# althonos/pyrodigal

Measured on AMD Instinct MI355X. Metric: Mbp/sec gene-called (meta mode), higher is better.
Workload: dtype f64; 1 GPU; 100000x20kbp_gc30-70_meta; contigs=100000, bases=2000000000, models=16, contigs_rank0=100000, sub_batch_contigs=6250, contexts_per_gpu=4, genes_all_ranks=2908995, steps_issued=a join of the contexts and a gather per step

## Files before the change

### pyrodigal_amd/csrc/finder.hip

```cpp
#include "pga_internal.h"
#include "pipeline.h"
#include "dpw_core.h"
#include "dev_common.h"

#include <math.h>
#include <stdio.h>
#include <stdlib.h>
#include <string.h>

#include <algorithm>
#include <atomic>
#include <chrono>
#include <condition_variable>
#include <functional>
#include <limits>
#include <map>
#include <memory>
#include <mutex>
#include <new>
#include <thread>
#include <type_traits>
#include <unordered_map>

namespace {
// ... 1511 lines not shown
                                  (int)batch->regions.size(), d_bits, d_mcounts, d_moff, d_miv, cap, st);
            HT(c, hipMemcpyAsync(h_moff_, d_moff, sizeof(int32_t) * (NC + 1), hipMemcpyDeviceToHost, st));
            h_moff = h_moff_; d_union_iv = d_miv;
            masks = MaskList{d_moff, d_miv};
        } else if (P.mask) {
            const int cap = (int)std::min<int64_t>(total / std::max(1, P.min_mask) + NC + 1, (int64_t)1 << 28);
            DEVBUF(d_runs, MaskRun, "d_mask_runs", cap + 1);
            DEVBUF(d_nruns, int32_t, "d_mask_count", 4);
            DEVBUF(d_moff, int32_t, "d_mask_off", NC + 2);
            DEVBUF(d_miv, int2, "d_mask_iv", cap + 1);
            pga_launch_find_masks(d_dig, d_ct, NC, batch->d_tiles, batch->n_tiles, P.min_mask, d_runs, d_nruns, cap, st);
            int32_t nruns = 0;
            HT(c, hipMemcpyAsync(&nruns, d_nruns, 4, hipMemcpyDeviceToHost, st));
            HT(c, hipStreamSynchronize(st));
            nruns = std::min(nruns, cap);
            std::vector<MaskRun> runs((size_t)nruns);
            if (nruns > 0) HT(c, hipMemcpy(runs.data(), d_runs, sizeof(MaskRun) * nruns, hipMemcpyDeviceToHost));
            std::sort(runs.begin(), runs.end(), [](const MaskRun& a, const MaskRun& b) { return a.contig != b.contig ? a.contig < b.contig : a.begin < b.begin; });
            std::vector<int32_t> moff(NC + 1, 0);
            std::vector<int2> miv((size_t)nruns + 1);
            for (int k = 0; k < nruns; k++) { moff[runs[k].contig + 1]++; miv[k] = make_int2(runs[k].begin, runs[k].end); }
            for (int i = 0; i < NC; i++) moff[i + 1] += moff[i];
            R->mask_off = moff;
            R->masks.resize(2 * (size_t)nruns);
            for (int k = 0; k < nruns; k++) { R->masks[2 * k] = runs[k].begin; R->masks[2 * k + 1] = runs[k].end; }
            HT(c, hipMemcpy(d_moff, moff.data(), sizeof(int32_t) * (NC + 1), hipMemcpyHostToDevice));
            if (nruns > 0) HT(c, hipMemcpy(d_miv, miv.data(), sizeof(int2) * nruns, hipMemcpyHostToDevice));
            masks = MaskList{d_moff, d_miv};
        }
        if (stage == PGA_STAGE_SEQUENCE) {
            HT(c, hipMemcpyAsync(h_cnt, d_cnt, sizeof(int32_t) * 2 * (size_t)NC, hipMemcpyDeviceToHost, st));
            HT(c, hipGetLastError());
            HT(c, hipStreamSynchronize(st));
            for (int i = 0; i < NC; i++) {
                R->contigs[i].gc = ct[i].len > 0 ? (double)h_cnt[i] / (double)ct[i].len : 0.0;
                R->contigs[i].n_unknown = h_cnt[NC + i];
            }
            if (h_moff) { const int rc = fetch_mask_union(c, R, h_moff, d_union_iv, NC); if (rc) return rc; }
            return publish(R, guard.r, P, out);
        }
        if (meta_run && NM > 0 && use_sets) {
            DEVBUF(d_set_of, int32_t, "d_set_of", 3 * (size_t)NC + 1);
            HT(c, hipMemcpyAsync(d_set_of, set_of.data(), sizeof(int32_t) * (size_t)NC, hipMemcpyHostToDevice, st));
            pga_launch_group_enable_sets(d_ct, NC, d_cnt, d_set_of, d_set_of + NC, f->d_model_gc, f->d_model_grp, NM, NG, d_enabled, st);
        } else if (meta_run && NM > 0) {
            pga_launch_group_enable(d_ct, NC, d_cnt, f->d_model_gc, f->d_model_grp, NM, NG, d_enabled, st);
        }
        if (multi) {
            for (int g = 0; g < NG; g++) for (int i = 0; i < NC; i++) h_enabled[(size_t)g * NC + i] = cgrp[i] == g;
            HT(c, hipMemcpyAsync(d_enabled, h_enabled, (size_t)NG * NC, hipMemcpyHostToDevice, st));
        }
        if (getenv("PGA_STAGE_FULL")) f->stage_full = true;
        bool stage_full = f->stage_full;
        c->extract_passes = 0;
        for (;;) {
            const bool half = !stage_full;
            const int shift = half ? std::max(1, std::min(8, getenv("PGA_STAGE_SHIFT") ? atoi(getenv("PGA_STAGE_SHIFT")) : 1)) : 0;
            const int64_t st_slots = half ? (total >> shift) + (int64_t)PGA_STAGE_SLACK * batch->n_tiles + 8 : 2 * total + 2;
            for (int g = 0; g < NG; g++) {
                char nm[32];
                GBUF(st_ndx, int32_t, st_slots) GBUF(st_sv, int32_t, st_slots) GBUF(st_info, uint8_t, st_slots)
                ga[g].st_half = shift; ga[g].st_overflow = d_st_overflow;
            }
            if (c->extract_passes > 0) HT(c, hipMemsetAsync(d_st_overflow, 0, sizeof(int32_t), st));
            for (int g = 0; g < NG; g++) {
                const int tt = meta_run ? f->group_tt[g] : multi ? gtt[g] : (stage == PGA_STAGE_EXTRACT ? tt_override : c->models[0].trans_table);
                pga_launch_extract(d_dig, total, d_ct, NC, tt, P, ga[g], batch->d_tiles, batch->n_tiles, batch->d_tile0, d_tile_first, d_tile_last,
                                   d_tile_count + (size_t)g * (batch->n_tiles + 1), d_tile_off + (size_t)g * (batch->n_tiles + 1), d_cbase + (size_t)g * (NC + 1),
                                   d_tile_scount + (size_t)g * (batch->n_tiles + 1), d_tile_soff + (size_t)g * (batch->n_tiles + 1), d_sbase + (size_t)g * (NC + 1),
                                   masks, st, ((meta_run && NM > 0) || multi) ? d_enabled + (size_t)g * NC : nullptr);
            }
            HT(c, hipMemcpyAsync(h_xa, d_xa, sizeof(int32_t) * xa_words, hipMemcpyDeviceToHost, st));
            HT(c, hipGetLastError());
            HT(c, hipStreamSynchronize(st));
            c->extract_passes++;
            if (!half || h_st_overflow[0] == 0) break;
            stage_full = true;
            if (!getenv("PGA_STAGE_SHIFT")) f->stage_full = true;
        }
        if (h_moff) { const int rc = fetch_mask_union(c, R, h_moff, d_union_iv, NC); if (rc) return rc; }

        tm.mark("extract+sync");
        int64_t group_nodes[4] = {0, 0, 0, 0};
        for (int g = 0; g < NG; g++) {
            char nm[32];
            group_nodes[g] = h_cbase[(size_t)g * (NC + 1) + NC];
            const int64_t n = group_nodes[g] + 1;
            GBUF(ndx, int32_t, n) GBUF(stop_val, int32_t, n) GBUF(type, uint8_t, n) GBUF(strand, int8_t, n) GBUF(edge0, uint8_t, n) GBUF(gc_cont, float, n) GBUF(contig_of, int32_t, n)
            GBUF(stop_list, int32_t, (int64_t)h_sbase[(size_t)g * (NC + 1) + NC] + 1)
            GBUF(start_list, int32_t, group_nodes[g] - (int64_t)h_sbase[(size_t)g * (NC + 1) + NC] + 1)
            GBUF(ovl_topo, uint32_t, (int64_t)h_sbase[(size_t)g * (NC + 1) + NC] + 1)
            GBUF(srank, int32_t, n + 4)
        }
        for (int g = 0; g < NG; g++) {
            pga_launch_place(d_ct, batch->d_tiles, batch->n_tiles, d_tile_off + (size_t)g * (batch->n_tiles + 1),
                             d_tile_soff + (size_t)g * (batch->n_tiles + 1), ga[g], st);
            pga_launch_orf_gc(d_ct, NC, d_dig, d_p16, ga[g], (int)group_nodes[g], d_cbase + (size_t)g * (NC + 1), st);
        }
        std::vector<std::vector<ChainDesc>> gch(NG);
        std::vector<double> mgc((size_t)NM); std::vector<int> mtt((size_t)NM);
        for (int m = 0; m < NM; m++) { mgc[m] = c->models[m].gc; mtt[m] = c->models[m].trans_table; }
        for (int g = 0; g < NG; g++) gch[g].reserve(meta_run ? (size_t)NC * 6 : (size_t)NC);
        std::vector<double> set_gc;
        if (use_sets) {
            std::vector<int64_t> sum((size_t)2 * NS, 0);
            for (int i = 0; i < NC; i++) { sum[2 * (size_t)set_of[i]] += h_cnt[i]; sum[2 * (size_t)set_of[i] + 1] += ct[i].len; }
            set_gc.resize((size_t)NS);
            for (int s = 0; s < NS; s++) set_gc[(size_t)s] = sum[2 * (size_t)s + 1] > 0 ? (double)sum[2 * (size_t)s] / (double)sum[2 * (size_t)s + 1] : 0.0;
        }
        for (int i = 0; i < NC; i++) {
            const int L = ct[i].len;
            double gc = L > 0 ? (double)h_cnt[i] / (double)L : 0.0;
            R->contigs[i].gc = gc;
            R->contigs[i].n_unknown = h_cnt[NC + i];
            if (!meta_run) {
                const int m = per_contig ? model_of_contig[i] : 0, g = multi ? cgrp[i] : 0;
                const int32_t* cb = h_cbase + (size_t)g * (NC + 1);
                ChainDesc ch{0, cb[i], cb[i + 1] - cb[i], m, i, 1};
                ch.group = g;
                gch[g].push_back(ch);
                continue;
            }
            if (use_sets) gc = set_gc[(size_t)set_of[i]];
            const double low = fmin(0.65, 0.88495 * gc - 0.0102337), high = fmax(0.35, 0.86596 * gc + 0.1131991);
            int tt_prev = -1;
            for (int m = 0; m < NM; m++) {
                if (mgc[m] < low || mgc[m] > high) continue;
                const int g = f->model_group[m];
                if (!h_enabled[(size_t)g * NC + i]) { c->err = "pga_find_genes: host and device disagree on a GC window"; return PGA_EDEVICE; }
                const int32_t* cb = h_cbase + (size_t)g * (NC + 1);
                ChainDesc ch{0, cb[i], cb[i + 1] - cb[i], m, i, mtt[m] != tt_prev ? 1 : 0};
// ... 1058 lines not shown
```

### pyrodigal_amd/csrc/pipeline.h

```cpp
#pragma once
#include "pga_internal.h"

struct ContigDesc {
    int64_t base;
    int32_t len;
    int32_t _pad;
};

#define PGA_STAGE_SLACK 8
struct TileDesc {
    int32_t contig;
    int32_t start;
};

struct GroupArrays {
    uint8_t* df;
    int32_t* c16; const int32_t* tile0 = nullptr;
    int32_t* st_ndx; int32_t* st_sv;
    uint8_t* st_info;
    int32_t st_half = 0; int32_t* st_overflow = nullptr;
    int32_t* stop_list;
    int32_t* start_list = nullptr;
    uint32_t* ovl_topo;
    int32_t* srank = nullptr;
    int32_t* ndx; int32_t* stop_val; uint8_t* type; int8_t* strand; uint8_t* edge0; float* gc_cont;
    int32_t* contig_of = nullptr;
};

struct ChainArrays {
    double* cscore; double* sscore; double* rscore; double* uscore; double* tscore; double* mot_score;
    double* cscore_raw;
    int32_t* star_ptr;
    int32_t* mot_ndx;
    uint8_t* rbs;
    uint8_t* edge;
    uint8_t* mot_len; uint8_t* mot_spacer; uint8_t* mot_spacendx;
    double* cs_sink = nullptr;
};

struct ModelScoreConst {
    double lfac_min, lfac_max;
    double lfac_tab[1001];
};

struct MaskList {
    const int32_t* off;
    const int2* iv;
};
struct MaskRun { int32_t contig, begin, end, _pad; };

struct ScoreParams {
    int32_t closed, is_meta, max_overlap, n_models;
    double* cs_out;
    uint8_t* conv_flag;
    unsigned long long* prof = nullptr;
    int32_t models_per_pass = 512;
    int32_t lean_stops = 0;
};

void pga_launch_digitize(const char* d_seq, uint8_t* d_dig, int64_t total, const ContigDesc* d_ct, int n_contigs,
                         int32_t* d_gc, int32_t* d_unk, hipStream_t st);
int64_t pga_gc_blocks(int64_t total);
void pga_launch_gc_prefix(const uint8_t* d_dig, int64_t total, int32_t* d_block_sum, int32_t* d_block_off, int32_t* d_p16, hipStream_t st);
void pga_launch_extract(const uint8_t* d_dig, int64_t total, const ContigDesc* d_ct, int n_contigs, int tt,
                        const pga_params& p, const GroupArrays& ga, const TileDesc* d_tiles, int n_tiles, const int32_t* d_tile0,
                        int32_t* d_tile_first, int32_t* d_tile_last, int32_t* d_tile_count, int32_t* d_tile_off, int32_t* d_cbase,
                        int32_t* d_tile_scount, int32_t* d_tile_soff, int32_t* d_sbase ,
                        MaskList masks, hipStream_t st,
                        const uint8_t* d_enabled = nullptr );
void pga_launch_place(const ContigDesc* d_ct, const TileDesc* d_tiles, int n_tiles, const int32_t* d_tile_off, const int32_t* d_tile_soff,
                      const GroupArrays& ga, hipStream_t st);
struct StopLaunch {
    const int32_t* sbase = nullptr;
    int64_t soff_begin = 0, n_pairs = 0;
    int32_t n_stops = 0;
    const int32_t* topo_q2 = nullptr; void* ext = nullptr;
    bool fill_star_ptr = true;
    bool starts_only = false; int32_t n_starts = 0;
    const int32_t* blk_chain = nullptr;
    void* mm_rec = nullptr;
    void* mm_chain = nullptr;
    void* mm_tile = nullptr;
    void* mm_scratch = nullptr;
    int32_t mm_tiles = 0;
};
int pga_mm_tile_items();
int32_t pga_mm_tiles(const ChainDesc* h_chains, int n_chains, const int32_t* h_cbase, const int32_t* h_sbase, int n_models, std::vector<int64_t>& scratch);
size_t pga_mm_scratch_bytes(int n_models, int n_chains);
constexpr size_t PGA_SS_REC_BYTES = 32, PGA_SS_MMCHAIN_BYTES = 32, PGA_SS_MMTILE_BYTES = 16;
void pga_launch_group_enable(const ContigDesc* d_ct, int n_contigs, const int32_t* d_gc_count, const double* d_model_gc,
                             const int32_t* d_model_group, int n_models, int n_groups, uint8_t* d_enabled, hipStream_t st);
void pga_launch_group_enable_sets(const ContigDesc* d_ct, int n_contigs, const int32_t* d_gc_count, const int32_t* d_set_of, int32_t* d_pool,
                                  const double* d_model_gc, const int32_t* d_model_group, int n_models, int n_groups, uint8_t* d_enabled,
                                  hipStream_t st);
void pga_launch_find_masks(const uint8_t* d_dig, const ContigDesc* d_ct, int n_contigs, const TileDesc* d_tiles, int n_tiles, int min_mask,
                           MaskRun* d_runs, int32_t* d_count, int cap, hipStream_t st);
int64_t pga_mask_words(int64_t total);
int64_t pga_mask_waves(int64_t total);
void pga_launch_mask_union(const uint8_t* d_dig, const char* d_seq, int64_t total, const ContigDesc* d_ct, int n_contigs, const TileDesc* d_tiles,
                           int n_tiles, int unknown_runs, int lower_case_runs, int min_mask, const MaskRun* d_regions, int n_regions,
                           uint32_t* d_bits, int32_t* d_counts, int32_t* d_moff, int2* d_miv, int cap, hipStream_t st);
int pga_extract_tile_size();
void pga_launch_orf_gc(const ContigDesc* d_ct, int n_contigs, const uint8_t* d_dig, const int32_t* d_p16, const GroupArrays& ga,
                       int n_nodes_total, const int32_t* d_node_contig_base, hipStream_t st);
void pga_launch_score(const ChainDesc* d_chains, int n_chains, int64_t node_begin, int64_t total, const uint8_t* d_dig,
                      const ContigDesc* d_ct, const GroupArrays& ga, const pga_training* d_models,
                      const ModelScoreConst* d_msc, const ModelConst* d_mc, const ChainArrays& ca, ScoreParams sp,
                      const ChainDesc* d_all_chains , const int2* d_contig_chains ,
                      const int32_t* d_node_contig_base, int n_contigs, int group_nodes, const unsigned* d_sd_lut, hipStream_t st,
                      int reuse_raw_cscore = 0 ,
                      const double* d_gil = nullptr , int il_stride = 0,
                      const int32_t* d_rank = nullptr ,
                      const void* d_cs_tasks = nullptr, int n_cs_tasks = 0, const void* d_cs_entries = nullptr ,
                      const StopLaunch* stops = nullptr);
bool pga_cs_tasks(const int2* h_cc, int n_contigs, const ChainDesc* h_chains, const int32_t* h_cbase, const int32_t* model_rank, int task_nodes,
                  std::vector<int32_t>& tasks, std::vector<int32_t>& entries);
void pga_launch_sd_lut(unsigned* d_lut, hipStream_t st);
```

### pyrodigal_amd/csrc/pipeline.hip

```cpp

#include "pga_internal.h"
#include "pipeline.h"
#include <atomic>
#include "dev_common.h"
#include "dpw_core.h"

namespace {

enum { NA = 0, NG = 1, NC = 2, NT = 3, NN = 6 };

__device__ __forceinline__ int find_contig(const ContigDesc* __restrict__ ct, int n, int64_t g) {
    int lo = 0, hi = n - 1;
    while (lo < hi) { int mid = (lo + hi + 1) >> 1; if (ct[mid].base <= g) lo = mid; else hi = mid - 1; }
    return lo;
}

__device__ __forceinline__ int block_contig(const ContigDesc* __restrict__ ct, int n, int64_t block_first, int64_t g, int* s_slot) {
    int c = block_search_le([&](const int k) { return ct[k].base; }, n, block_first, s_slot);
    while (c + 1 < n && ct[c + 1].base <= g) c++;
    return c;
}
__device__ __forceinline__ int block_chain(const ChainDesc* __restrict__ ch, int n, int64_t block_first, int64_t g, int* s_slot) {
    int c = block_search_le([&](const int k) { return ch[k].off; }, n, block_first, s_slot);
    while (c + 1 < n && ch[c + 1].off <= g) c++;
// ... 108 lines not shown
            int a = in ? gc : 0, u = in ? unk : 0;
#pragma unroll
            for (int m = 32; m >= 1; m >>= 1) { a += __shfl_xor(a, m, 64); u += __shfl_xor(u, m, 64); }
            if (acc_c != c0) {
                if ((threadIdx.x & 63) == 0 && acc_c >= 0) { if (acc_gc) atomicAdd(&gc_count[acc_c], acc_gc); if (acc_unk) atomicAdd(&unk_count[acc_c], acc_unk); }
                acc_c = c0; acc_gc = 0; acc_unk = 0;
            }
            acc_gc += a; acc_unk += u;
        } else if (in && one_contig) {
            if (gc) atomicAdd(&gc_count[c], gc);
            if (unk) atomicAdd(&unk_count[c], unk);
        }
    }
    __shared__ int s_c[4], s_g[4], s_u[4];
    const int wv = threadIdx.x >> 6;
    if ((threadIdx.x & 63) == 0) { s_c[wv] = acc_c; s_g[wv] = acc_gc; s_u[wv] = acc_unk; }
    __syncthreads();
    if (threadIdx.x == 0) {
#pragma unroll
        for (int w = 0; w < 4; w++) {
            if (s_c[w] < 0) continue;
            int g = s_g[w], u = s_u[w];
#pragma unroll
            for (int v = w + 1; v < 4; v++) if (s_c[v] == s_c[w]) { g += s_g[v]; u += s_u[v]; s_c[v] = -1; }
            if (g) atomicAdd(&gc_count[s_c[w]], g);
            if (u) atomicAdd(&unk_count[s_c[w]], u);
        }
    }
}

constexpr int EX_TILE = 3072;
constexpr int EX_PER_THREAD = 12;
constexpr int EX_NONE_HI = 0x7fffffff;

__device__ __forceinline__ unsigned pack4(const unsigned w, const bool comp) {
    unsigned c = w & 0x03030303u;
    if (comp) { const unsigned nm = (w >> 2) & 0x01010101u; c = (c ^ 0x03030303u) ^ (nm | (nm << 1)); }
    return (c | (c >> 6) | (c >> 12) | (c >> 18)) & 0xffu;
}
__device__ __forceinline__ unsigned long long pack16(const uint4 v, const bool comp) {
    return (unsigned long long)(pack4(v.x, comp) | (pack4(v.y, comp) << 8) | (pack4(v.z, comp) << 16) | (pack4(v.w, comp) << 24));
}
__device__ __forceinline__ unsigned long long pairrev64(unsigned long long x) {
    x = __brevll(x);
    return ((x & 0x5555555555555555ull) << 1) | ((x >> 1) & 0x5555555555555555ull);
}

struct TileGeom {
    int L, a, len;
    __device__ __forceinline__ int lo(const int strand) const { return strand == 1 ? a : L - a - len; }
};
__device__ __forceinline__ TileGeom tile_geom(const TileDesc td, const int L) { return TileGeom{L, td.start, min(EX_TILE, L - td.start)}; }

struct ExShared {
    int lsc[3][256];
    int scm[256];
    int32_t sv[2][EX_PER_THREAD][256];
    int wmin[3][4], wmax[3][4], wlsc[3][4];
    int carry_ns[3], carry_ps[3];
    int wsum[4];
};

struct ExParams { int tt, closed, min_gene, min_edge_gene; unsigned long long stop_codons, start_codons; };

__device__ __forceinline__ unsigned pairrev32(unsigned x) {
    x = __brev(x);
    return ((x & 0x55555555u) << 1) | ((x >> 1) & 0x55555555u);
}
__device__ __forceinline__ unsigned unknown4(const unsigned w) {
    const unsigned n = (w >> 2) & 0x01010101u;
    return (n | (n >> 7) | (n >> 14) | (n >> 21)) & 0xfu;
}

template <int STRAND>
__device__ __forceinline__ void strand_codon_masks(const TileGeom G, const uint8_t* __restrict__ d, const int64_t base, const int64_t total, const int i0,
                                                   const unsigned long long stop_codons, const unsigned long long start_codons,
                                                   unsigned& inm, unsigned& cw, unsigned& stm, unsigned& scm) {
    constexpr bool FWD = STRAND == 1;
    const int L = G.L, lo = G.lo(STRAND), end = lo + G.len;
    const int qa = max(0, lo - i0), qb = min(EX_PER_THREAD - 1, min(end - 1, L - 3) - i0);
    inm = qb >= qa ? ((2u << qb) - 1u) & ~((1u << qa) - 1u) : 0u;
    cw = 0; unsigned unk = 0xffffu;
    if (inm) {
        const int64_t ga0 = FWD ? base + i0 : base + (L - 1 - i0 - 15);
        if (ga0 >= 0 && ga0 <= total) {
            uint4 v; __builtin_memcpy(&v, (FWD ? d + i0 : d + (L - 1 - i0 - 15)), 16);
            const unsigned q0 = (unsigned)pack16(v, !FWD);
            const unsigned n0 = unknown4(v.x) | (unknown4(v.y) << 4) | (unknown4(v.z) << 8) | (unknown4(v.w) << 12);
            cw = FWD ? q0 : pairrev32(q0);
            unk = FWD ? n0 : (__brev(n0) >> 16);
        } else {
            unk = 0;
            for (int q = 0; q < 16; q++) {
                const int i = i0 + q;
                const int b = (i >= 0 && i < L) ? sbase(d, L, i, STRAND) : NN;
                if (b > 3) unk |= 1u << q; else cw |= (unsigned)b << (2 * q);
            }
        }
        if (i0 < 0) unk |= (1u << min(16, -i0)) - 1u;
        if (i0 + 16 > L) unk |= ~((1u << max(0, L - i0)) - 1u) & 0xffffu;
    }
    stm = 0; scm = 0;
#pragma unroll
    for (int q = 0; q < EX_PER_THREAD; q++) {
        const unsigned idx = (cw >> (2 * q)) & 63u;
        stm |= ((unsigned)(stop_codons >> idx) & 1u) << q;
        scm |= ((unsigned)(start_codons >> idx) & 1u) << q;
    }
    const unsigned okm = inm & ~(unk | (unk >> 1) | (unk >> 2));
    stm &= okm; scm &= okm;
}

template <int STRAND>
__device__ __forceinline__ void extract_strand(ExShared& S, const TileGeom G, const uint8_t* __restrict__ d, const int64_t base, const int64_t total,
                                               const int tile, const TileDesc* __restrict__ tiles, const int n_tiles,
                                               const int32_t* __restrict__ tile_first, const int32_t* __restrict__ tile_last, const ExParams P,
                                               const int n_masks, const int2* __restrict__ mv, unsigned& nodes, unsigned long long& infos) {
    constexpr bool FWD = STRAND == 1;
    const int t = threadIdx.x, lane = t & 63, w = t >> 6, L = G.L, s = FWD ? 0 : 1;
    const int lo = G.lo(STRAND), end = lo + G.len;
    const int top = FWD ? G.a : L - 1 - G.a - (EX_PER_THREAD - 1);
    const int i0 = FWD ? top + t * EX_PER_THREAD : top - t * EX_PER_THREAD;
    const int f0 = ((top % 3) + 3) % 3;
    nodes = 0; infos = 0;
    if (t < 6) {
        const int f = t % 3;
        const int64_t so = (int64_t)s * n_tiles;
        const int contig = tiles[tile].contig;
        const int up = FWD ? 1 : -1;
        if (t < 3) {
            int v = EX_NONE_HI;
            for (int k = tile + up; k >= 0 && k < n_tiles && tiles[k].contig == contig; k += up) {
                v = tile_first[(so + k) * 3 + f];
                if (v != EX_NONE_HI) break;
            }
            S.carry_ns[f] = v;
        } else {
            int v = -1;
            for (int k = tile - up; k >= 0 && k < n_tiles && tiles[k].contig == contig; k -= up) {
                v = tile_last[(so + k) * 3 + f];
                if (v != -1) break;
            }
            S.carry_ps[f] = v;
        }
    }
    unsigned inm, cw, stm, scm;
    strand_codon_masks<STRAND>(G, d, base, total, i0, P.stop_codons, P.start_codons, inm, cw, stm, scm);
    int mn[3], mx[3], ls[3];
#pragma unroll
    for (int r = 0; r < 3; r++) {
        const unsigned fr = 0x249u << r;
        const unsigned a = stm & fr, b = scm & fr;
        mn[r] = a ? i0 + __builtin_ctz(a) : EX_NONE_HI;
        mx[r] = a ? i0 + 31 - __builtin_clz(a) : -1;
        ls[r] = b ? i0 + 31 - __builtin_clz(b) : -1;
    }
    const unsigned long long lanes_up = FWD ? (~1ull << lane) : ((1ull << lane) - 1ull);
    const unsigned long long lanes_dn = FWD ? ((1ull << lane) - 1ull) : (~1ull << lane);
    int xa[3], xb[3], xe[3];
#pragma unroll
    for (int r = 0; r < 3; r++) {
        const unsigned long long hs = __ballot(mx[r] >= 0), hc = __ballot(ls[r] >= 0);
        const unsigned long long mu = hs & lanes_up, md = hs & lanes_dn, mc = hc & lanes_dn;
        const int su = mu ? (FWD ? __builtin_ctzll(mu) : 63 - __builtin_clzll(mu)) : lane;
        const int sd = md ? (FWD ? 63 - __builtin_clzll(md) : __builtin_ctzll(md)) : lane;
        const int sc = mc ? (FWD ? 63 - __builtin_clzll(mc) : __builtin_ctzll(mc)) : lane;
        const int va = __shfl(mn[r], su, 64), vb = __shfl(mx[r], sd, 64), ve = __shfl(ls[r], sc, 64);
        xa[r] = mu ? va : EX_NONE_HI;
        xb[r] = md ? vb : -1;
        xe[r] = ls[r] >= 0 ? ls[r] : (mc ? ve : -1);
        const int l_first = hs ? (FWD ? __builtin_ctzll(hs) : 63 - __builtin_clzll(hs)) : 0;
        const int l_last = hs ? (FWD ? 63 - __builtin_clzll(hs) : __builtin_ctzll(hs)) : 0;
        const int l_lastc = hc ? (FWD ? 63 - __builtin_clzll(hc) : __builtin_ctzll(hc)) : 0;
        const int w_mn = __shfl(mn[r], l_first, 64), w_mx = __shfl(mx[r], l_last, 64), w_ls = __shfl(ls[r], l_lastc, 64);
        if (lane == 0) { S.wmin[r][w] = hs ? w_mn : EX_NONE_HI; S.wmax[r][w] = hs ? w_mx : -1; S.wlsc[r][w] = hc ? w_ls : -1; }
    }
    S.scm[t] = (int)scm;
    __syncthreads();
    int nxt[3], prv[3];
#pragma unroll
    for (int r = 0; r < 3; r++) {
        int a = xa[r], b = xb[r], e = xe[r];
#pragma unroll
        for (int k = 0; k < 4; k++) {
            const bool up_side = FWD ? k > w : k < w, dn_side = FWD ? k < w : k > w;
            if (up_side) a = min(a, S.wmin[r][k]);
            if (dn_side) { b = max(b, S.wmax[r][k]); e = max(e, S.wlsc[r][k]); }
        }
        const int f = (f0 + r) % 3;
        nxt[r] = a == EX_NONE_HI ? S.carry_ns[f] : a;
        prv[r] = b == -1 ? S.carry_ps[f] : b;
        S.lsc[r][t] = e;
    }
    __syncthreads();
    auto mask_bound = [&](const int last) -> int {
        if (n_masks <= 0) return INT_MIN;
        if (FWD) {
            int a = 0, b = n_masks;
            while (a < b) { const int m = (a + b) >> 1; if (mv[m].x <= last) a = m + 1; else b = m; }
            if (a > 0) { const int2 m = mv[a - 1]; if (m.x < last) return m.y; }
        } else {
            const int x = L - last - 1;
            int a = 0, b = n_masks;
            while (a < b) { const int m = (a + b) >> 1; if (mv[m].y < x) a = m + 1; else b = m; }
            if (a < n_masks) { const int2 m = mv[a]; if (x < m.y) return L - 1 - m.x; }
        }
        return INT_MIN;
    };
    auto last_start_codon = [&](const int r, const int f, const int x, const int lower) -> int {
        int y;
        if (x >= lo) {
            const int tx = FWD ? (x - top) / EX_PER_THREAD : (top + EX_PER_THREAD - 1 - x) / EX_PER_THREAD;
            const int i0x = FWD ? top + tx * EX_PER_THREAD : top - tx * EX_PER_THREAD;
            const unsigned m = (unsigned)S.scm[tx] & ((2u << (x - i0x)) - 1u) & (0x249u << r);
            if (m) return i0x + 31 - __builtin_clz(m);
            const int nb = FWD ? tx - 1 : tx + 1;
            const int v = (nb >= 0 && nb < 256) ? S.lsc[r][nb] : -1;
            if (v >= 0) return v;
            y = lo - 1 - ((lo - 1 - f) % 3 + 3) % 3;
        } else y = x - ((x - f) % 3 + 3) % 3;
        for (int i = y; i >= lower && i >= 0; i -= 3)
            if (codon_is_start(sbase(d, L, i, STRAND), sbase(d, L, i + 1, STRAND), sbase(d, L, i + 2, STRAND), P.tt)) return i;
        return -1;
    };
    auto orf_has_start = [&](const int r, const int f, const int last, const int left, const bool real) -> bool {
        const int mb = mask_bound(last);
        const int lower = max(left + 1, mb);
        const int mind = real ? P.min_gene : P.min_edge_gene;
        const int x = min(last + 3 - mind, last - 3);
        if (x >= lower && last_start_codon(r, f, x, lower) >= lower) return true;
        return !P.closed && left < 0 && f < last && last - f > P.min_edge_gene && f >= mb;
    };
    auto put = [&](const int q, const int info, const int sv) {
        const int k = FWD ? q : EX_PER_THREAD - 1 - q;
        nodes |= 1u << k;
        infos |= (unsigned long long)info << (4 * k);
        S.sv[s][k][t] = sv;
    };
    unsigned cand = stm | scm;
    if (!P.closed) {
        if (i0 <= 2 && i0 + EX_PER_THREAD > 0) cand |= (i0 >= 0 ? 7u >> i0 : 7u << -i0) & inm;
#pragma unroll
        for (int r = 0; r < 3; r++) {
            const int f = (f0 + r) % 3;
            const int q = (L - 3 - ((L - 3 - f) % 3)) - i0;
            if (q >= 0 && q < EX_PER_THREAD) cand |= (1u << q) & inm;
        }
    }
    auto candidate = [&](const int q, const bool is_stop) {
        const int i = i0 + q;
        const int r = q % 3, f = (f0 + r) % 3;
        const unsigned fr = 0x249u << r;
        const unsigned above = stm & fr & ~((2u << q) - 1u);
        const unsigned below = stm & fr & ((1u << q) - 1u);
        const int left = below ? i0 + 31 - __builtin_clz(below) : (r == 0 ? prv[0] : (r == 1 ? prv[1] : prv[2]));
        const int sv_stop = FWD ? (left >= 0 ? left : f - 6) : (left >= 0 ? L - 1 - left : L - f + 5);
        if (is_stop) {
            if (orf_has_start(r, f, i, left, true)) put(q, PGA_T_STOP, sv_stop);
            return;
        }
        int last = above ? i0 + __builtin_ctz(above) : (r == 0 ? nxt[0] : (r == 1 ? nxt[1] : nxt[2]));
        const bool real = last != EX_NONE_HI;
        if (!real) {
            if (P.closed) return;
            last = L - 3 - ((L - 3 - f) % 3);
            if (last < i) return;
            if (last == i) {
                if (orf_has_start(r, f, i, left, false)) put(q, PGA_T_STOP | (1 << 2), sv_stop);
                return;
            }
        }
        if (n_masks > 0 && i < mask_bound(last)) return;
        const int mind = real ? P.min_gene : P.min_edge_gene;
        int type = -1, edge = 0;
        const int c0 = (int)((cw >> (2 * q)) & 3u);
        if (last - i + 3 >= mind && ((scm >> q) & 1u)) type = c0 == NA ? 0 : (c0 == NT ? 2 : 1);
        else if (i <= 2 && !P.closed && last - i > P.min_edge_gene) { type = 0; edge = 1; }
        if (type < 0) return;
        put(q, type | (edge << 2), FWD ? last : L - 1 - last);
    };
    unsigned stops = stm;
    while (stops) { const int q = __builtin_ctz(stops); stops &= stops - 1u; candidate(q, true); }
    cand &= ~stm;
    while (cand) { const int q = __builtin_ctz(cand); cand &= cand - 1u; candidate(q, false); }
}

__global__ void __launch_bounds__(64)
k_tile_stops(const uint8_t* __restrict__ dig, int64_t total, const ContigDesc* __restrict__ ct, const TileDesc* __restrict__ tiles, int n_tiles,
             unsigned long long stop_codons, int32_t* __restrict__ tile_first, int32_t* __restrict__ tile_last, const uint8_t* __restrict__ enabled) {
    const TileDesc td = tiles[blockIdx.x];
    if (enabled != nullptr && !enabled[td.contig]) return;
    const ContigDesc cd = ct[td.contig];
    const TileGeom G = tile_geom(td, cd.len);
    const int lane = threadIdx.x & 63, hl = lane & 31;
    const bool first = lane < 32;
    const uint8_t* __restrict__ d = dig + cd.base;
    constexpr int CHUNK = 32 * EX_PER_THREAD;
#pragma unroll
    for (int s = 0; s < 2; s++) {
        const int lo = G.lo(s == 0 ? 1 : -1), end = lo + G.len;
        int res[3];
        res[0] = res[1] = res[2] = first ? EX_NONE_HI : -1;
        unsigned found = 0;
        int fbase = 0;
        for (int c = 0; c * CHUNK < G.len && found != 63u; c++) {
            const int i0 = first ? lo + c * CHUNK + hl * EX_PER_THREAD : end - c * CHUNK - (hl + 1) * EX_PER_THREAD;
            fbase = ((i0 % 3) + 3) % 3;
            unsigned inm, cw, stm, scm;
            if (s == 0) strand_codon_masks<1>(G, d, cd.base, total, i0, stop_codons, 0ull, inm, cw, stm, scm);
            else strand_codon_masks<-1>(G, d, cd.base, total, i0, stop_codons, 0ull, inm, cw, stm, scm);
#pragma unroll
            for (int r = 0; r < 3; r++) {
                const unsigned m = stm & (0x249u << r);
                const unsigned long long hs = __ballot(m != 0u);
                const unsigned h_first = (unsigned)hs, h_last = (unsigned)(hs >> 32);
                const int v = m ? (first ? i0 + __builtin_ctz(m) : i0 + 31 - __builtin_clz(m)) : 0;
                const int src = first ? (h_first ? __builtin_ctz(h_first) : 0) : (h_last ? 32 + __builtin_ctz(h_last) : 32);
                const int wv = __shfl(v, src, 64);
                const bool mine_has = first ? h_first != 0u : h_last != 0u;
                const unsigned bit = first ? (1u << r) : (8u << r);
                if (mine_has && !(found & bit)) res[r] = wv;
                found |= (h_first ? (1u << r) : 0u) | (h_last ? (8u << r) : 0u);
            }
        }
        if (hl < 3) {
            const int f = (fbase + hl) % 3;
            const int64_t o = ((int64_t)s * n_tiles + blockIdx.x) * 3 + f;
            const int v = hl == 0 ? res[0] : (hl == 1 ? res[1] : res[2]);
            if (first) tile_first[o] = v; else tile_last[o] = v;
        }
    }
}

__global__ void __launch_bounds__(256)
k_extract_tile(const uint8_t* __restrict__ dig, int64_t total, const ContigDesc* __restrict__ ct, const TileDesc* __restrict__ tiles, int n_tiles,
               const int32_t* __restrict__ tile_first, const int32_t* __restrict__ tile_last, ExParams P, GroupArrays ga, MaskList masks,
               const uint8_t* __restrict__ enabled, int32_t* __restrict__ tile_count, int32_t* __restrict__ tile_scount) {
    __shared__ ExShared S;
    __shared__ int s_stops;
    const int tile = blockIdx.x, t = threadIdx.x;
    const TileDesc td = tiles[tile];
    if (enabled != nullptr && !enabled[td.contig]) { if (t == 0) { tile_count[tile] = 0; tile_scount[tile] = 0; } return; }
    if (t == 0) s_stops = 0;
    const ContigDesc cd = ct[td.contig];
    const TileGeom G = tile_geom(td, cd.len);
    const uint8_t* __restrict__ d = dig + cd.base;
    const int n_masks = masks.off ? masks.off[td.contig + 1] - masks.off[td.contig] : 0;
    const int2* __restrict__ mv = masks.off ? masks.iv + masks.off[td.contig] : nullptr;
    unsigned nf, nr; unsigned long long inf_f, inf_r;
    extract_strand<1>(S, G, d, cd.base, total, tile, tiles, n_tiles, tile_first, tile_last, P, n_masks, mv, nf, inf_f);
    __syncthreads();
    extract_strand<-1>(S, G, d, cd.base, total, tile, tiles, n_tiles, tile_first, tile_last, P, n_masks, mv, nr, inf_r);
    const int r0 = t * EX_PER_THREAD;
    const int cnt = __popc(nf) + __popc(nr);
    int inc = cnt;
    const int lane = t & 63, w = t >> 6;
#pragma unroll
    for (int off = 1; off < 64; off <<= 1) { const int v = __shfl_up(inc, off, 64); if (lane >= off) inc += v; }
    if (lane == 63) S.wsum[w] = inc;
    __syncthreads();
    int nbase = inc - cnt;
    for (int k = 0; k < w; k++) nbase += S.wsum[k];
    if (t == 255) tile_count[tile] = nbase + cnt;
    const int64_t g0 = cd.base + G.a;
    if (r0 < G.len) {
        const int nk = min(EX_PER_THREAD, G.len - r0);
        auto spread4 = [](const unsigned x) { return ((x & 15u) * 0x00204081u) & 0x01010101u; };
        if (nk == EX_PER_THREAD) {
            unsigned w[3];
            __builtin_memcpy(w, dig + g0 + r0, 12);
#pragma unroll
            for (int q = 0; q < 3; q++) w[q] = (w[q] & 0x07070707u) | (spread4(nf >> (4 * q)) << 4) | (spread4(nr >> (4 * q)) << 5);
            __builtin_memcpy(ga.df + g0 + r0, w, 12);
        } else {
            for (int k = 0; k < nk; k++) ga.df[g0 + r0 + k] = (uint8_t)((dig[g0 + r0 + k] & 7u) | (((nf >> k) & 1u) << 4) | (((nr >> k) & 1u) << 5));
        }
    }
    const int64_t stage0 = ga.st_half ? (g0 >> ga.st_half) + (int64_t)PGA_STAGE_SLACK * tile : 2 * g0;
    const int room = ga.st_half ? (G.len >> ga.st_half) + PGA_STAGE_SLACK : 2 * G.len;
    if (t == 255 && nbase + cnt > room) atomicOr(ga.st_overflow, 1);
    int64_t slot = stage0 + nbase;
    const int64_t slot_end = stage0 + room;
    unsigned both = nf | nr;
    int n_stop = 0;
    while (both) {
        const int k = __builtin_ctz(both);
        both &= both - 1u;
        if ((nf >> k) & 1u) {
            const int info = (int)((inf_f >> (4 * k)) & 7);
            if (slot < slot_end) { ga.st_ndx[slot] = G.a + r0 + k; ga.st_sv[slot] = S.sv[0][k][t]; ga.st_info[slot] = (uint8_t)info; }
            slot++; n_stop += (info & 3) == PGA_T_STOP;
        }
        if ((nr >> k) & 1u) {
            const int info = (int)((inf_r >> (4 * k)) & 7);
            if (slot < slot_end) { ga.st_ndx[slot] = G.a + r0 + k; ga.st_sv[slot] = S.sv[1][k][t]; ga.st_info[slot] = (uint8_t)(info | 8); }
            slot++; n_stop += (info & 3) == PGA_T_STOP;
        }
    }
#pragma unroll
    for (int m = 32; m >= 1; m >>= 1) n_stop += __shfl_xor(n_stop, m, 64);
    if (lane == 0 && n_stop) atomicAdd(&s_stops, n_stop);
    __syncthreads();
    if (t == 0) tile_scount[tile] = s_stops;
}

constexpr int SCAN_E = 4;
__device__ __forceinline__ int scan_pad(const int i) { return i + (i >> 5); }
__global__ void __launch_bounds__(1024)
k_scan_counts(const int32_t* __restrict__ cnt, int n, int32_t* __restrict__ off, const int32_t* __restrict__ cnt2, int32_t* __restrict__ off2) {
    __shared__ int s_a[SCAN_E * 1024 + SCAN_E * 32], s_b[SCAN_E * 1024 + SCAN_E * 32];
    __shared__ int s_w[16], s_w2[16];
    __shared__ int s_carry, s_carry2;
    const int t = threadIdx.x, lane = t & 63, w = t >> 6;
    const bool two = cnt2 != nullptr;
    if (t == 0) { s_carry = 0; s_carry2 = 0; }
    __syncthreads();
    for (int base = 0; base < n; base += SCAN_E * 1024) {
        int c[SCAN_E], c2[SCAN_E];
#pragma unroll
        for (int k = 0; k < SCAN_E; k++) {
            const int g = base + k * 1024 + t;
            c[k] = g < n ? cnt[g] : 0;
            c2[k] = two && g < n ? cnt2[g] : 0;
        }
#pragma unroll
        for (int k = 0; k < SCAN_E; k++) { s_a[scan_pad(k * 1024 + t)] = c[k]; s_b[scan_pad(k * 1024 + t)] = c2[k]; }
        __syncthreads();
        int v[SCAN_E], v2[SCAN_E], sum = 0, sum2 = 0;
#pragma unroll
        for (int k = 0; k < SCAN_E; k++) { v[k] = s_a[scan_pad(t * SCAN_E + k)]; v2[k] = s_b[scan_pad(t * SCAN_E + k)]; sum += v[k]; sum2 += v2[k]; }
        int inc = sum, inc2 = sum2;
#pragma unroll
        for (int o = 1; o < 64; o <<= 1) {
            const int x = __shfl_up(inc, o, 64), x2 = __shfl_up(inc2, o, 64);
            if (lane >= o) { inc += x; inc2 += x2; }
        }
        if (lane == 63) { s_w[w] = inc; s_w2[w] = inc2; }
        __syncthreads();
        int run = s_carry + inc - sum, run2 = s_carry2 + inc2 - sum2;
        for (int k = 0; k < w; k++) { run += s_w[k]; run2 += s_w2[k]; }
#pragma unroll
        for (int k = 0; k < SCAN_E; k++) {
            s_a[scan_pad(t * SCAN_E + k)] = run; s_b[scan_pad(t * SCAN_E + k)] = run2;
            run += v[k]; run2 += v2[k];
        }
        __syncthreads();
#pragma unroll
        for (int k = 0; k < SCAN_E; k++) {
// ... 2133 lines not shown
#pragma unroll
    for (int o = 1; o < 64; o <<= 1) {
        const int x = __shfl_up(is, o, 64), y = __shfl_up(ie, o, 64);
        if (lane >= o) { is += x; ie += y; }
    }
    if (!(S | E)) return;
    int ks = off_s[w >> 6] + is - ns, ke = off_e[w >> 6] + ie - ne;
    while (S) {
        const int64_t g = w * 32 + __builtin_ctz(S);
        S &= S - 1u;
        if (ks < cap) iv[ks].x = (int)(g - ct[find_contig(ct, n_contigs, g)].base);
        ks++;
    }
    while (E) {
        const int64_t g = w * 32 + __builtin_ctz(E);
        E &= E - 1u;
        if (ke < cap) iv[ke].y = (int)(g + 1 - ct[find_contig(ct, n_contigs, g)].base);
        ke++;
    }
}

int64_t pga_mask_words(int64_t total) { return (total + 32) / 32; }
int64_t pga_mask_waves(int64_t total) { return (pga_mask_words(total) + 63) / 64; }

void pga_launch_mask_union(const uint8_t* d_dig, const char* d_seq, int64_t total, const ContigDesc* d_ct, int n_contigs, const TileDesc* d_tiles,
                           int n_tiles, int unknown_runs, int lower_case_runs, int min_mask, const MaskRun* d_regions, int n_regions,
                           uint32_t* d_bits, int32_t* d_counts, int32_t* d_moff, int2* d_miv, int cap, hipStream_t st) {
    const int64_t nw = pga_mask_words(total), nwv = pga_mask_waves(total);
    uint32_t* const d_cbits = d_bits + nw;
    int32_t* const cnt_s = d_counts; int32_t* const cnt_e = cnt_s + (nwv + 1); int32_t* const off_s = cnt_e + (nwv + 1); int32_t* const off_e = off_s + (nwv + 1);
    (void)hipMemsetAsync(d_bits, 0, sizeof(uint32_t) * 2 * (size_t)nw, st);
    const dim3 run_grid(n_tiles + (n_contigs + 255) / 256);
    if (unknown_runs) hipLaunchKernelGGL(k_mask_paint_runs<RunOfUnknown>, run_grid, dim3(256), 0, st, d_dig, d_ct, d_tiles, n_tiles, n_contigs, min_mask, d_bits);
    if (lower_case_runs) hipLaunchKernelGGL(k_mask_paint_runs<RunOfLowerCase>, run_grid, dim3(256), 0, st, (const uint8_t*)d_seq, d_ct, d_tiles, n_tiles, n_contigs, min_mask, d_bits);
    hipLaunchKernelGGL(k_mask_paint_regions, dim3((n_regions + 3) / 4 + (n_contigs + 255) / 256), dim3(256), 0, st, d_regions, n_regions, d_ct, n_contigs, d_bits, d_cbits);
    const int word_blocks = (int)((nw + 255) / 256);
    hipLaunchKernelGGL(k_mask_count, dim3(word_blocks), dim3(256), 0, st, (const uint32_t*)d_bits, (const uint32_t*)d_cbits, nw, cnt_s, cnt_e);
    hipLaunchKernelGGL(k_scan_counts, dim3(1), dim3(1024), 0, st, (const int32_t*)cnt_s, (int)nwv, off_s, (const int32_t*)cnt_e, off_e);
    hipLaunchKernelGGL(k_mask_place, dim3(word_blocks + (n_contigs + 1 + 255) / 256), dim3(256), 0, st, (const uint32_t*)d_bits, (const uint32_t*)d_cbits, nw, word_blocks,
                       (const int32_t*)off_s, (const int32_t*)off_e, d_ct, n_contigs, d_moff, d_miv, cap);
}

void pga_launch_gc_prefix(const uint8_t* d_dig, int64_t total, int32_t* d_block_sum, int32_t* d_block_off, int32_t* d_p16, hipStream_t st) {
    if (total <= 0) return;
    const int nb = (int)pga_gc_blocks(total);
    hipLaunchKernelGGL(k_gcp_blocks, dim3(nb), dim3(256), 0, st, d_dig, total, d_block_sum);
    hipLaunchKernelGGL(k_scan_counts, dim3(1), dim3(1024), 0, st, d_block_sum, nb, d_block_off, (const int32_t*)nullptr, (int32_t*)nullptr);
    hipLaunchKernelGGL(k_gcp_final, dim3(nb), dim3(256), 0, st, d_dig, total, d_block_off, d_p16);
}

void pga_launch_extract(const uint8_t* d_dig, int64_t total, const ContigDesc* d_ct, int n_contigs, int tt,
                        const pga_params& p, const GroupArrays& ga, const TileDesc* d_tiles, int n_tiles, const int32_t* d_tile0,
                        int32_t* d_tile_first, int32_t* d_tile_last, int32_t* d_tile_count, int32_t* d_tile_off, int32_t* d_cbase,
                        int32_t* d_tile_scount, int32_t* d_tile_soff, int32_t* d_sbase, MaskList masks, hipStream_t st, const uint8_t* d_enabled) {
    if (n_tiles > 0) {
        ExParams P{tt, p.closed, p.min_gene, p.min_edge_gene, 0ull, 0ull};
        for (int idx = 0; idx < 64; idx++) {
            const int b0 = idx & 3, b1 = (idx >> 2) & 3, b2 = (idx >> 4) & 3;
            if (codon_is_stop(b0, b1, b2, tt)) P.stop_codons |= 1ull << idx;
            if (codon_is_start(b0, b1, b2, tt)) P.start_codons |= 1ull << idx;
        }
        hipLaunchKernelGGL(k_tile_stops, dim3(n_tiles), dim3(64), 0, st, d_dig, total, d_ct, d_tiles, n_tiles, P.stop_codons, d_tile_first, d_tile_last, d_enabled);
        hipLaunchKernelGGL(k_extract_tile, dim3(n_tiles), dim3(256), 0, st, d_dig, total, d_ct, d_tiles, n_tiles, d_tile_first, d_tile_last, P, ga, masks,
                           d_enabled, d_tile_count, d_tile_scount);
    }
    hipLaunchKernelGGL(k_scan_counts, dim3(1), dim3(1024), 0, st, d_tile_count, n_tiles, d_tile_off, (const int32_t*)d_tile_scount, d_tile_soff);
    hipLaunchKernelGGL(k_contig_node_base, dim3((n_contigs + 1 + 255) / 256), dim3(256), 0, st, d_tile0, n_contigs, d_tile_off, d_cbase);
    hipLaunchKernelGGL(k_contig_node_base, dim3((n_contigs + 1 + 255) / 256), dim3(256), 0, st, d_tile0, n_contigs, d_tile_soff, d_sbase);
}

void pga_launch_place(const ContigDesc* d_ct, const TileDesc* d_tiles, int n_tiles, const int32_t* d_tile_off, const int32_t* d_tile_soff,
                      const GroupArrays& ga, hipStream_t st) {
    if (n_tiles <= 0) return;
    hipLaunchKernelGGL(k_place_nodes, dim3(n_tiles), dim3(128), 0, st, d_ct, d_tiles, d_tile_off, d_tile_soff, ga);
}

int pga_extract_tile_size() { return EX_TILE; }

bool pga_cs_tasks(const int2* h_cc , int n_contigs, const ChainDesc* h_chains, const int32_t* h_cbase,
                  const int32_t* model_rank, int task_nodes, std::vector<int32_t>& tasks , std::vector<int32_t>& entries ) {
    tasks.clear(); entries.clear();
    std::vector<std::vector<int32_t>> bucket(64);
    for (int i = 0; i < n_contigs; i++) {
        const int2 cc = h_cc[i];
        if (cc.y <= 0 || h_cbase[i + 1] == h_cbase[i]) continue;
        const int r0 = model_rank[h_chains[cc.x].model];
        for (int m = 1; m < cc.y; m++) if (model_rank[h_chains[cc.x + m].model] != r0 + m) return false;
        for (int m0 = 0; m0 < cc.y; m0 += 4) {
            if (r0 + m0 >= 64) return false;
            bucket[(size_t)(r0 + m0)].push_back(i); bucket[(size_t)(r0 + m0)].push_back(m0);
        }
    }
    for (int q = 63; q >= 0; q--) {
        const std::vector<int32_t>& b = bucket[(size_t)q];
        int first = (int)(entries.size() / 4), count = 0, nodes = 0, cuts = 0;
        auto flush = [&]() {
            if (count > 0) { tasks.push_back(q); tasks.push_back(first); tasks.push_back(count); tasks.push_back(0); }
            first += count; count = 0; nodes = 0; cuts = 0;
        };
        for (size_t k = 0; k < b.size(); k += 2) {
            const int nc = h_cbase[b[k] + 1] - h_cbase[b[k]];
            for (int f0 = 0; f0 < nc; f0 += task_nodes) {
                const int piece = std::min(task_nodes, nc - f0);
                if (count > 0 && (nodes + piece > task_nodes || count == CS_TASK_MAX_ENTRIES || (piece != nc && cuts == CS_TASK_MAX_CUTS))) flush();
                entries.push_back(b[k]); entries.push_back(b[k + 1]); entries.push_back(f0); entries.push_back(piece);
                count++; nodes += piece; cuts += piece != nc;
            }
        }
        flush();
    }
    return true;
}

__global__ void __launch_bounds__(256)
k_group_enable(const ContigDesc* __restrict__ ct, int n_contigs, const int32_t* __restrict__ gc_count, const double* __restrict__ model_gc,
               const int32_t* __restrict__ model_group, int n_models, int n_groups, uint8_t* __restrict__ enabled ) {
    const int i = blockIdx.x * blockDim.x + threadIdx.x;
// ... 193 lines not shown
```

Before: 21160 Mbp/s.

## Compact extract-tile shared stop-value storage with overflow pool to raise occupancy

```diff
diff --git a/pyrodigal_amd/csrc/finder.hip b/pyrodigal_amd/csrc/finder.hip
--- a/pyrodigal_amd/csrc/finder.hip
+++ b/pyrodigal_amd/csrc/finder.hip
@@ -1587,6 +1587,8 @@
         }
         if (getenv("PGA_STAGE_FULL")) f->stage_full = true;
         bool stage_full = f->stage_full;
+        int ex_c = getenv("PGA_EXTRACT_C") ? std::max(0, std::min(4, atoi(getenv("PGA_EXTRACT_C")))) : 4;
+        const int ex_pool = getenv("PGA_EXTRACT_POOL") ? std::max(0, std::min(128, atoi(getenv("PGA_EXTRACT_POOL")))) : 128;
         c->extract_passes = 0;
         for (;;) {
             const bool half = !stage_full;
@@ -1603,15 +1605,19 @@
                 pga_launch_extract(d_dig, total, d_ct, NC, tt, P, ga[g], batch->d_tiles, batch->n_tiles, batch->d_tile0, d_tile_first, d_tile_last,
                                    d_tile_count + (size_t)g * (batch->n_tiles + 1), d_tile_off + (size_t)g * (batch->n_tiles + 1), d_cbase + (size_t)g * (NC + 1),
                                    d_tile_scount + (size_t)g * (batch->n_tiles + 1), d_tile_soff + (size_t)g * (batch->n_tiles + 1), d_sbase + (size_t)g * (NC + 1),
-                                   masks, st, ((meta_run && NM > 0) || multi) ? d_enabled + (size_t)g * NC : nullptr);
+                                   masks, st, ((meta_run && NM > 0) || multi) ? d_enabled + (size_t)g * NC : nullptr, ex_c, ex_pool);
             }
             HT(c, hipMemcpyAsync(h_xa, d_xa, sizeof(int32_t) * xa_words, hipMemcpyDeviceToHost, st));
             HT(c, hipGetLastError());
             HT(c, hipStreamSynchronize(st));
             c->extract_passes++;
-            if (!half || h_st_overflow[0] == 0) break;
-            stage_full = true;
-            if (!getenv("PGA_STAGE_SHIFT")) f->stage_full = true;
+            const bool staging_overflow = half && (h_st_overflow[0] & 1), pool_exhausted = ex_c > 0 && (h_st_overflow[0] & 2);
+            if (!staging_overflow && !pool_exhausted) break;
+            if (pool_exhausted) ex_c = 0;
+            if (staging_overflow) {
+                stage_full = true;
+                if (!getenv("PGA_STAGE_SHIFT")) f->stage_full = true;
+            }
         }
         if (h_moff) { const int rc = fetch_mask_union(c, R, h_moff, d_union_iv, NC); if (rc) return rc; }
 
diff --git a/pyrodigal_amd/csrc/pipeline.h b/pyrodigal_amd/csrc/pipeline.h
--- a/pyrodigal_amd/csrc/pipeline.h
+++ b/pyrodigal_amd/csrc/pipeline.h
@@ -67,7 +67,9 @@
                         int32_t* d_tile_first, int32_t* d_tile_last, int32_t* d_tile_count, int32_t* d_tile_off, int32_t* d_cbase,
                         int32_t* d_tile_scount, int32_t* d_tile_soff, int32_t* d_sbase ,
                         MaskList masks, hipStream_t st,
-                        const uint8_t* d_enabled = nullptr );
+                        const uint8_t* d_enabled = nullptr ,
+                        int ex_c = 4 ,
+                        int ex_pool = 128 );
 void pga_launch_place(const ContigDesc* d_ct, const TileDesc* d_tiles, int n_tiles, const int32_t* d_tile_off, const int32_t* d_tile_soff,
                       const GroupArrays& ga, hipStream_t st);
 struct StopLaunch {
diff --git a/pyrodigal_amd/csrc/pipeline.hip b/pyrodigal_amd/csrc/pipeline.hip
--- a/pyrodigal_amd/csrc/pipeline.hip
+++ b/pyrodigal_amd/csrc/pipeline.hip
@@ -184,16 +184,58 @@
 };
 __device__ __forceinline__ TileGeom tile_geom(const TileDesc td, const int L) { return TileGeom{L, td.start, min(EX_TILE, L - td.start)}; }
 
+constexpr int EX_C = 4;
+constexpr int EX_POOL = 128;
+constexpr unsigned EX_IN_POOL = 15u;
+template <bool COMPACT>
 struct ExShared {
     int lsc[3][256];
-    int scm[256];
-    int32_t sv[2][EX_PER_THREAD][256];
+    uint16_t scm[256];
+    int32_t sv[2][COMPACT ? EX_C : EX_PER_THREAD][256];
+    int32_t pool_key[COMPACT ? EX_POOL : 1], pool_sv[COMPACT ? EX_POOL : 1];
+    int pool_n;
     int wmin[3][4], wmax[3][4], wlsc[3][4];
-    int carry_ns[3], carry_ps[3];
+    int carry_ns[2][3], carry_ps[2][3];
     int wsum[4];
 };
 
-struct ExParams { int tt, closed, min_gene, min_edge_gene; unsigned long long stop_codons, start_codons; };
+struct ExParams { int tt, closed, min_gene, min_edge_gene; unsigned long long stop_codons, start_codons; int ex_c, ex_pool; };
+
+struct ExCarry { int k, step, v, same; };
+__device__ __forceinline__ ExCarry carry_begin(const int t, const int tile, const int contig, const TileDesc* __restrict__ tiles, const int n_tiles,
+                                               const int32_t* __restrict__ tile_first, const int32_t* __restrict__ tile_last) {
+    ExCarry c{0, 0, 0, 0};
+    if (t < 12) {
+        const int s = t / 6, f = t % 3;
+        const bool ns = t % 6 < 3;
+        const int up = s == 0 ? 1 : -1;
+        c.step = ns ? up : -up;
+        c.k = tile + c.step;
+        c.v = ns ? EX_NONE_HI : -1;
+        if (c.k >= 0 && c.k < n_tiles) {
+            c.same = tiles[c.k].contig == contig;
+            c.v = (ns ? tile_first : tile_last)[((int64_t)s * n_tiles + c.k) * 3 + f];
+        }
+    }
+    return c;
+}
+template <bool COMPACT>
+__device__ __forceinline__ void carry_finish(ExShared<COMPACT>& S, ExCarry c, const int t, const int contig, const TileDesc* __restrict__ tiles, const int n_tiles,
+                                             const int32_t* __restrict__ tile_first, const int32_t* __restrict__ tile_last) {
+    if (t < 12) {
+        const int s = t / 6, f = t % 3;
+        const bool ns = t % 6 < 3;
+        const int none = ns ? EX_NONE_HI : -1;
+        const int32_t* __restrict__ arr = ns ? tile_first : tile_last;
+        if (!c.same) c.v = none;
+        else while (c.v == none) {
+            c.k += c.step;
+            if (c.k < 0 || c.k >= n_tiles || tiles[c.k].contig != contig) break;
+            c.v = arr[((int64_t)s * n_tiles + c.k) * 3 + f];
+        }
+        if (ns) S.carry_ns[s][f] = c.v; else S.carry_ps[s][f] = c.v;
+    }
+}
 
 __device__ __forceinline__ unsigned pairrev32(unsigned x) {
     x = __brev(x);
@@ -243,39 +285,19 @@
     stm &= okm; scm &= okm;
 }
 
-template <int STRAND>
-__device__ __forceinline__ void extract_strand(ExShared& S, const TileGeom G, const uint8_t* __restrict__ d, const int64_t base, const int64_t total,
-                                               const int tile, const TileDesc* __restrict__ tiles, const int n_tiles,
+template <int STRAND, bool COMPACT>
+__device__ __forceinline__ void extract_strand(ExShared<COMPACT>& S, const TileGeom G, const uint8_t* __restrict__ d, const int64_t base, const int64_t total,
+                                               const int contig, const TileDesc* __restrict__ tiles, const int n_tiles,
                                                const int32_t* __restrict__ tile_first, const int32_t* __restrict__ tile_last, const ExParams P,
-                                               const int n_masks, const int2* __restrict__ mv, unsigned& nodes, unsigned long long& infos) {
+                                               const int n_masks, const int2* __restrict__ mv, const ExCarry carry,
+                                               unsigned& nodes, unsigned long long& infos, unsigned long long& slots) {
     constexpr bool FWD = STRAND == 1;
     const int t = threadIdx.x, lane = t & 63, w = t >> 6, L = G.L, s = FWD ? 0 : 1;
     const int lo = G.lo(STRAND), end = lo + G.len;
     const int top = FWD ? G.a : L - 1 - G.a - (EX_PER_THREAD - 1);
     const int i0 = FWD ? top + t * EX_PER_THREAD : top - t * EX_PER_THREAD;
     const int f0 = ((top % 3) + 3) % 3;
-    nodes = 0; infos = 0;
-    if (t < 6) {
-        const int f = t % 3;
-        const int64_t so = (int64_t)s * n_tiles;
-        const int contig = tiles[tile].contig;
-        const int up = FWD ? 1 : -1;
-        if (t < 3) {
-            int v = EX_NONE_HI;
-            for (int k = tile + up; k >= 0 && k < n_tiles && tiles[k].contig == contig; k += up) {
-                v = tile_first[(so + k) * 3 + f];
-                if (v != EX_NONE_HI) break;
-            }
-            S.carry_ns[f] = v;
-        } else {
-            int v = -1;
-            for (int k = tile - up; k >= 0 && k < n_tiles && tiles[k].contig == contig; k -= up) {
-                v = tile_last[(so + k) * 3 + f];
-                if (v != -1) break;
-            }
-            S.carry_ps[f] = v;
-        }
-    }
+    nodes = 0; infos = 0; slots = 0;
     unsigned inm, cw, stm, scm;
     strand_codon_masks<STRAND>(G, d, base, total, i0, P.stop_codons, P.start_codons, inm, cw, stm, scm);
     int mn[3], mx[3], ls[3];
@@ -307,7 +329,8 @@
         const int w_mn = __shfl(mn[r], l_first, 64), w_mx = __shfl(mx[r], l_last, 64), w_ls = __shfl(ls[r], l_lastc, 64);
         if (lane == 0) { S.wmin[r][w] = hs ? w_mn : EX_NONE_HI; S.wmax[r][w] = hs ? w_mx : -1; S.wlsc[r][w] = hc ? w_ls : -1; }
     }
-    S.scm[t] = (int)scm;
+    S.scm[t] = (uint16_t)scm;
+    if (FWD) carry_finish(S, carry, t, contig, tiles, n_tiles, tile_first, tile_last);
     __syncthreads();
     int nxt[3], prv[3];
 #pragma unroll
@@ -320,8 +343,8 @@
             if (dn_side) { b = max(b, S.wmax[r][k]); e = max(e, S.wlsc[r][k]); }
         }
         const int f = (f0 + r) % 3;
-        nxt[r] = a == EX_NONE_HI ? S.carry_ns[f] : a;
-        prv[r] = b == -1 ? S.carry_ps[f] : b;
+        nxt[r] = a == EX_NONE_HI ? S.carry_ns[s][f] : a;
+        prv[r] = b == -1 ? S.carry_ps[s][f] : b;
         S.lsc[r][t] = e;
     }
     __syncthreads();
@@ -365,9 +388,19 @@
     };
     auto put = [&](const int q, const int info, const int sv) {
         const int k = FWD ? q : EX_PER_THREAD - 1 - q;
+        if constexpr (COMPACT) {
+            const int n = __popc(nodes);
+            if (n < P.ex_c) {
+                S.sv[s][n][t] = sv;
+                slots |= (unsigned long long)n << (4 * k);
+            } else {
+                slots |= (unsigned long long)EX_IN_POOL << (4 * k);
+                const int e = atomicAdd(&S.pool_n, 1);
+                if (e < P.ex_pool) { S.pool_key[e] = t | (s << 8) | (k << 9); S.pool_sv[e] = sv; }
+            }
+        } else S.sv[s][k][t] = sv;
         nodes |= 1u << k;
         infos |= (unsigned long long)info << (4 * k);
-        S.sv[s][k][t] = sv;
     };
     unsigned cand = stm | scm;
     if (!P.closed) {
@@ -464,25 +497,36 @@
     }
 }
 
-__global__ void __launch_bounds__(256)
+template <bool COMPACT>
+__global__ void __launch_bounds__(256, COMPACT ? 8 : 5)
 k_extract_tile(const uint8_t* __restrict__ dig, int64_t total, const ContigDesc* __restrict__ ct, const TileDesc* __restrict__ tiles, int n_tiles,
                const int32_t* __restrict__ tile_first, const int32_t* __restrict__ tile_last, ExParams P, GroupArrays ga, MaskList masks,
                const uint8_t* __restrict__ enabled, int32_t* __restrict__ tile_count, int32_t* __restrict__ tile_scount) {
-    __shared__ ExShared S;
+    __shared__ ExShared<COMPACT> S;
     __shared__ int s_stops;
     const int tile = blockIdx.x, t = threadIdx.x;
     const TileDesc td = tiles[tile];
     if (enabled != nullptr && !enabled[td.contig]) { if (t == 0) { tile_count[tile] = 0; tile_scount[tile] = 0; } return; }
-    if (t == 0) s_stops = 0;
+    const ExCarry carry = carry_begin(t, tile, td.contig, tiles, n_tiles, tile_first, tile_last);
+    if (t == 0) { s_stops = 0; S.pool_n = 0; }
     const ContigDesc cd = ct[td.contig];
     const TileGeom G = tile_geom(td, cd.len);
     const uint8_t* __restrict__ d = dig + cd.base;
     const int n_masks = masks.off ? masks.off[td.contig + 1] - masks.off[td.contig] : 0;
     const int2* __restrict__ mv = masks.off ? masks.iv + masks.off[td.contig] : nullptr;
-    unsigned nf, nr; unsigned long long inf_f, inf_r;
-    extract_strand<1>(S, G, d, cd.base, total, tile, tiles, n_tiles, tile_first, tile_last, P, n_masks, mv, nf, inf_f);
+    unsigned nf, nr; unsigned long long inf_f, inf_r, sl_f, sl_r;
+    extract_strand<1>(S, G, d, cd.base, total, td.contig, tiles, n_tiles, tile_first, tile_last, P, n_masks, mv, carry, nf, inf_f, sl_f);
     __syncthreads();
-    extract_strand<-1>(S, G, d, cd.base, total, tile, tiles, n_tiles, tile_first, tile_last, P, n_masks, mv, nr, inf_r);
+    extract_strand<-1>(S, G, d, cd.base, total, td.contig, tiles, n_tiles, tile_first, tile_last, P, n_masks, mv, carry, nr, inf_r, sl_r);
+    auto stop_val_at = [&](const int s, const int k, const unsigned long long sl) -> int32_t {
+        if constexpr (COMPACT) {
+            const unsigned slot = (unsigned)(sl >> (4 * k)) & 15u;
+            if (slot != EX_IN_POOL) return S.sv[s][slot][t];
+            const int key = t | (s << 8) | (k << 9), n = min(S.pool_n, P.ex_pool);
+            for (int e = 0; e < n; e++) if (S.pool_key[e] == key) return S.pool_sv[e];
+            return 0;
+        } else return S.sv[s][k][t];
+    };
     const int r0 = t * EX_PER_THREAD;
     const int cnt = __popc(nf) + __popc(nr);
     int inc = cnt;
@@ -511,6 +555,7 @@
     const int64_t stage0 = ga.st_half ? (g0 >> ga.st_half) + (int64_t)PGA_STAGE_SLACK * tile : 2 * g0;
     const int room = ga.st_half ? (G.len >> ga.st_half) + PGA_STAGE_SLACK : 2 * G.len;
     if (t == 255 && nbase + cnt > room) atomicOr(ga.st_overflow, 1);
+    if (COMPACT && t == 0 && S.pool_n > P.ex_pool) atomicOr(ga.st_overflow, 2);
     int64_t slot = stage0 + nbase;
     const int64_t slot_end = stage0 + room;
     unsigned both = nf | nr;
@@ -520,12 +565,12 @@
         both &= both - 1u;
         if ((nf >> k) & 1u) {
             const int info = (int)((inf_f >> (4 * k)) & 7);
-            if (slot < slot_end) { ga.st_ndx[slot] = G.a + r0 + k; ga.st_sv[slot] = S.sv[0][k][t]; ga.st_info[slot] = (uint8_t)info; }
+            if (slot < slot_end) { ga.st_ndx[slot] = G.a + r0 + k; ga.st_sv[slot] = stop_val_at(0, k, sl_f); ga.st_info[slot] = (uint8_t)info; }
             slot++; n_stop += (info & 3) == PGA_T_STOP;
         }
         if ((nr >> k) & 1u) {
             const int info = (int)((inf_r >> (4 * k)) & 7);
-            if (slot < slot_end) { ga.st_ndx[slot] = G.a + r0 + k; ga.st_sv[slot] = S.sv[1][k][t]; ga.st_info[slot] = (uint8_t)(info | 8); }
+            if (slot < slot_end) { ga.st_ndx[slot] = G.a + r0 + k; ga.st_sv[slot] = stop_val_at(1, k, sl_r); ga.st_info[slot] = (uint8_t)(info | 8); }
             slot++; n_stop += (info & 3) == PGA_T_STOP;
         }
     }
@@ -2765,17 +2810,22 @@
 void pga_launch_extract(const uint8_t* d_dig, int64_t total, const ContigDesc* d_ct, int n_contigs, int tt,
                         const pga_params& p, const GroupArrays& ga, const TileDesc* d_tiles, int n_tiles, const int32_t* d_tile0,
                         int32_t* d_tile_first, int32_t* d_tile_last, int32_t* d_tile_count, int32_t* d_tile_off, int32_t* d_cbase,
-                        int32_t* d_tile_scount, int32_t* d_tile_soff, int32_t* d_sbase, MaskList masks, hipStream_t st, const uint8_t* d_enabled) {
+                        int32_t* d_tile_scount, int32_t* d_tile_soff, int32_t* d_sbase, MaskList masks, hipStream_t st, const uint8_t* d_enabled,
+                        int ex_c, int ex_pool) {
     if (n_tiles > 0) {
-        ExParams P{tt, p.closed, p.min_gene, p.min_edge_gene, 0ull, 0ull};
+        ExParams P{tt, p.closed, p.min_gene, p.min_edge_gene, 0ull, 0ull, std::min(ex_c, EX_C), std::max(0, std::min(ex_pool, EX_POOL))};
         for (int idx = 0; idx < 64; idx++) {
             const int b0 = idx & 3, b1 = (idx >> 2) & 3, b2 = (idx >> 4) & 3;
             if (codon_is_stop(b0, b1, b2, tt)) P.stop_codons |= 1ull << idx;
             if (codon_is_start(b0, b1, b2, tt)) P.start_codons |= 1ull << idx;
         }
         hipLaunchKernelGGL(k_tile_stops, dim3(n_tiles), dim3(64), 0, st, d_dig, total, d_ct, d_tiles, n_tiles, P.stop_codons, d_tile_first, d_tile_last, d_enabled);
-        hipLaunchKernelGGL(k_extract_tile, dim3(n_tiles), dim3(256), 0, st, d_dig, total, d_ct, d_tiles, n_tiles, d_tile_first, d_tile_last, P, ga, masks,
-                           d_enabled, d_tile_count, d_tile_scount);
+        if (P.ex_c > 0)
+            hipLaunchKernelGGL(k_extract_tile<true>, dim3(n_tiles), dim3(256), 0, st, d_dig, total, d_ct, d_tiles, n_tiles, d_tile_first, d_tile_last, P, ga, masks,
+                               d_enabled, d_tile_count, d_tile_scount);
+        else
+            hipLaunchKernelGGL(k_extract_tile<false>, dim3(n_tiles), dim3(256), 0, st, d_dig, total, d_ct, d_tiles, n_tiles, d_tile_first, d_tile_last, P, ga, masks,
+                               d_enabled, d_tile_count, d_tile_scount);
     }
     hipLaunchKernelGGL(k_scan_counts, dim3(1), dim3(1024), 0, st, d_tile_count, n_tiles, d_tile_off, (const int32_t*)d_tile_scount, d_tile_soff);
     hipLaunchKernelGGL(k_contig_node_base, dim3((n_contigs + 1 + 255) / 256), dim3(256), 0, st, d_tile0, n_contigs, d_tile_off, d_cbase);
```

New measurement: 22090 Mbp/s, median of 6. 1.04x the previous value.
